# kchmck/p25rx

Measured on NVIDIA B200. Metric: Msamples/s IQ demod+decode (real-time P25 channels = baseband samples/s / 48000), higher is better.
Workload: dtype f32

## Files before the change

### p25rx_b200/csrc/ddc_fm.cu

```cuda
#include <stdlib.h>

#include "p25cu_internal.cuh"
#include "p25_imma_tables.h"

__constant__ float c_taps_front[P25_TAPS_FRONT];
__constant__ float c_taps_decim[P25_TAPS_DECIM];
__constant__ float c_taps_chan[P25_TAPS_CHAN];
__constant__ float c_iq_lut[256];

static_assert(P25_TAPS_FRONT == 5 * P25_DECIM_FRONT, "front stage is a 10-phase x 5-tap polyphase matrix");
static_assert(P25_TAPS_DECIM == 5 * P25_DECIM_NATIVE, "decimator is a 5-phase x 5-tap polyphase matrix");

template <bool FRONT>
struct Cfg {
    static constexpr int MB = FRONT ? 64 : 256;
    static constexpr int NT = FRONT ? 320 : 256;
    static constexpr int DIN = FRONT ? 50 : 5;
    static constexpr int XN = MB * DIN;
    static constexpr int ACOLS = FRONT ? 5 * MB : 0;
    static constexpr int RING = FRONT ? 128 : 512;
    static constexpr int HT = FRONT ? 3264 : 1312;
};

template <bool FRONT>
// ... 1462 lines not shown
      }
      if (it_first + n_st == ips) {
          const uint4* src = reinterpret_cast<const uint4*>(chunk + ((size_t)p.n - p.ht) * ES);
          uint4* dst = reinterpret_cast<uint4*>((unsigned char*)p.tail_out + s * tail_bytes);
          for (int i = lane; i < (int)(tail_bytes / 16); i += 32) dst[i] = src[i];
      }
      s++;
      it_first = 0;
      chunk += row_bytes;
      tail += tail_bytes;
    }
}

using Tables = p25imma::Tables5;
static_assert(NB == p25imma::NB5 && SCALE_LOG2 == p25imma::SCALE5 && sizeof(g_btab) == sizeof(Tables::b), "table geometry");
static const Tables& tables() {
    static const Tables t(P25_TAPS_DECIM_H);
    return t;
}

}


namespace w50i {

using fast::mbar_init;
using fast::mbar_expect_tx;
using fast::mbar_wait;
using fast::tma_load_1d;
using fast::cfma;
using fast5::add2;
using fast5::disc_atan2_pair;
using w5i::imma;
using w5i::imma0;
using w5i::lds32;

constexpr int D = 50;
constexpr int G = P25_TAPS_FRONT + P25_DECIM_FRONT * (P25_TAPS_DECIM - 1);
constexpr int R = 4;
constexpr int NOUT = 32 * R;
constexpr int XNEW = D * NOUT;
constexpr int XREAD = D * (NOUT - 1) + G;
constexpr int WARPS = 12;
constexpr int AL = 8, ES = 2;
constexpr int XLEN = (XREAD + 2 * AL - 2) / AL * AL;
constexpr int KS = 28;
// ... 233 lines not shown

unsigned p25cu_ddc_tail_len(int decimation) { return decimation == 50 ? Cfg<true>::HT : Cfg<false>::HT; }

cudaError_t p25cu_ddc_upload_taps() {
    cudaError_t e;
    if ((e = cudaMemcpyToSymbol(c_taps_front, P25_TAPS_FRONT_H, sizeof(c_taps_front))) != cudaSuccess) return e;
    if ((e = cudaMemcpyToSymbol(c_taps_decim, P25_TAPS_DECIM_H, sizeof(c_taps_decim))) != cudaSuccess) return e;
    if ((e = cudaMemcpyToSymbol(c_taps_chan, P25_TAPS_CHAN_H, sizeof(c_taps_chan))) != cudaSuccess) return e;
    {
        const w5i::Tables& t = w5i::tables();
        if (!t.ok) return cudaErrorInvalidValue;
        if ((e = cudaMemcpyToSymbol(w5i::g_btab, t.b, sizeof(w5i::g_btab))) != cudaSuccess) return e;
        const int4 q[3] = {make_int4(t.init[0], t.init[0], t.init[0], t.init[0]), make_int4(t.init[1], t.init[1], t.init[1], t.init[1]),
                           make_int4(t.init[2], t.init[2], t.init[2], t.init[2])};
        if ((e = cudaMemcpyToSymbol(w5i::g_init, q, sizeof(q))) != cudaSuccess) return e;
    }
    {
        const w50i::Tables& t = w50i::tables();
        if (!t.ok) return cudaErrorInvalidValue;
        if ((e = cudaMemcpyToSymbol(w50i::g_btab, t.b, sizeof(w50i::g_btab))) != cudaSuccess) return e;
        const int4 q[3] = {make_int4(t.init[0], t.init[0], t.init[0], t.init[0]), make_int4(t.init[1], t.init[1], t.init[1], t.init[1]),
                           make_int4(t.init[2], t.init[2], t.init[2], t.init[2])};
        if ((e = cudaMemcpyToSymbol(w50i::g_init, q, sizeof(q))) != cudaSuccess) return e;
    }
    return cudaMemcpyToSymbol(c_iq_lut, P25_IQ_LUT, sizeof(c_iq_lut));
}

template <bool FRONT, int FMT>
static cudaError_t launch(const DdcParams& p, cudaStream_t st) {
    using C = Cfg<FRONT>;
    auto kern = p25_ddc_fm_kernel<FRONT, FMT>;
    const size_t smem = sizeof(Smem<FRONT>);
    kern<<<p.n_streams * p.n_seg, C::NT, smem, st>>>(p);
    return cudaGetLastError();
}

unsigned p25cu_ddc_block_out(int decimation) { return decimation == 50 ? Cfg<true>::MB : Cfg<false>::MB; }

static double tap_gain(const float* h, int n) {
    double g = 0.0;
    for (int k = 0; k < n; k++) g += (double)h[k];
    return g;
}

template <int FMT>
static cudaError_t launch_fast(const DdcParams& p, cudaStream_t st) {
// ... 42 lines not shown
    const unsigned grid = want < (unsigned long long)grid_max ? (unsigned)(want ? want : 1) : (unsigned)grid_max;
    const bool u8 = FMT == P25CU_FMT_U8_IQ;
    const float dc = u8 ? (float)(0.5 * tap_gain(P25_TAPS_DECIM_H, P25_TAPS_DECIM) * tap_gain(P25_TAPS_CHAN_H, P25_TAPS_CHAN)) : 0.f;
    kern<<<grid, 32 * w5::WARPS, smem, st>>>(p, ips, dc, u8 ? (float)(1.0 / (127.5 * 127.5)) : 1.f);
    return cudaGetLastError();
}

static cudaError_t launch_w5i(const DdcParams& p, cudaStream_t st) {
    const size_t smem = sizeof(w5i::WarpSm) * w5i::WARPS + sizeof(uint2) * w5i::NB * 32;
    const unsigned ips = (p.n_out + w5i::NOUT - 1) / w5i::NOUT;
    const unsigned long long total = (unsigned long long)p.n_streams * ips;
    unsigned long long want = (total + 3) / 4;
    want = (want + w5i::WARPS - 1) / w5i::WARPS;
    const unsigned grid = want < (unsigned long long)p.plan->grid_w5i ? (unsigned)(want ? want : 1) : (unsigned)p.plan->grid_w5i;
    const w5i::Tables& t = w5i::tables();
    const double sc = (double)(1 << w5i::SCALE_LOG2);
    const float dc = (float)(0.5 * t.gain * tap_gain(P25_TAPS_CHAN_H, P25_TAPS_CHAN) * sc);
    const float pw_scale = (float)(1.0 / (127.5 * 127.5) / (sc * sc));
    if (p.power_sum) w5i::p25_ddc5_imma_kernel<true><<<grid, 32 * w5i::WARPS, smem, st>>>(p, ips, dc, pw_scale);
    else w5i::p25_ddc5_imma_kernel<false><<<grid, 32 * w5i::WARPS, smem, st>>>(p, ips, dc, pw_scale);
    return cudaGetLastError();
}

static cudaError_t launch_w50i(const DdcParams& p, cudaStream_t st) {
    const size_t smem = sizeof(w50i::WarpSm) * w50i::WARPS + sizeof(uint2) * w50i::NB * 32;
    const unsigned ips = (p.n_out + w50i::NOUT - 1) / w50i::NOUT;
    const unsigned long long total = (unsigned long long)p.n_streams * ips;
    unsigned long long want = (total + 3) / 4;
    want = (want + w50i::WARPS - 1) / w50i::WARPS;
    const unsigned grid = want < (unsigned long long)p.plan->grid_w50i ? (unsigned)(want ? want : 1) : (unsigned)p.plan->grid_w50i;
    const w50i::Tables& t = w50i::tables();
    const double sc = (double)(1 << w50i::SCALE_LOG2);
    const float dc = (float)(0.5 * t.gain * tap_gain(P25_TAPS_CHAN_H, P25_TAPS_CHAN) * sc);
    const float pw_scale = (float)(1.0 / (127.5 * 127.5) / (sc * sc));
    if (p.power_sum) w50i::p25_ddc50_imma_kernel<true><<<grid, 32 * w50i::WARPS, smem, st>>>(p, ips, dc, pw_scale);
    else w50i::p25_ddc50_imma_kernel<false><<<grid, 32 * w50i::WARPS, smem, st>>>(p, ips, dc, pw_scale);
    return cudaGetLastError();
}

template <typename K>
static cudaError_t plan_one(K kern, int threads, size_t smem, int n_sm, int* grid) {
    cudaError_t e = cudaFuncSetAttribute(kern, cudaFuncAttributeMaxDynamicSharedMemorySize, (int)smem);
    if (e != cudaSuccess) return e;
    int per_sm = 0;
    e = cudaOccupancyMaxActiveBlocksPerMultiprocessor(&per_sm, kern, threads, smem);
    if (e != cudaSuccess) return e;
// ... 6 lines not shown
    const int n_sm = plan->n_sm;
    constexpr int U8 = P25CU_FMT_U8_IQ, CF = P25CU_FMT_CF32_IQ;
    if ((e = plan_one(fast::p25_ddc_fm_stream_kernel<CF>, fast::NT, sizeof(fast::Smem<CF>), n_sm, &plan->grid_ddc50)) != cudaSuccess) return e;
    if ((e = plan_one(fast::p25_ddc_fm_stream_kernel<U8>, fast::NT, sizeof(fast::Smem<U8>), n_sm, &plan->grid_ddc50_u8)) != cudaSuccess) return e;
    if (const char* ev = getenv("P25CU_DDC_CTAS")) {
        const int per_sm = atoi(ev);
        if (per_sm > 0) plan->grid_ddc50 = plan->grid_ddc50_u8 = n_sm * per_sm;
    }
    if ((e = plan_one(fast5::p25_ddc5_fm_kernel<U8>, fast5::K<U8>::NT, sizeof(fast5::Smem<U8>), n_sm, &plan->grid_fast5[U8])) != cudaSuccess) return e;
    if ((e = plan_one(fast5::p25_ddc5_fm_kernel<CF>, fast5::K<CF>::NT, sizeof(fast5::Smem<CF>), n_sm, &plan->grid_fast5[CF])) != cudaSuccess) return e;
    if ((e = plan_one(w5::p25_ddc5_warp_kernel<U8, false>, 32 * w5::WARPS, sizeof(w5::WarpSm<U8>) * w5::WARPS, n_sm, &plan->grid_w5[U8])) != cudaSuccess) return e;
    if ((e = plan_one(w5::p25_ddc5_warp_kernel<CF, false>, 32 * w5::WARPS, sizeof(w5::WarpSm<CF>) * w5::WARPS, n_sm, &plan->grid_w5[CF])) != cudaSuccess) return e;
    if (const char* ev = getenv("P25CU_W5_CTAS")) {
        const int per_sm = atoi(ev);
        if (per_sm > 0) plan->grid_w5[U8] = plan->grid_w5[CF] = n_sm * per_sm;
    }
    const size_t smem_w5i = sizeof(w5i::WarpSm) * w5i::WARPS + sizeof(uint2) * w5i::NB * 32;
    if ((e = plan_one(w5i::p25_ddc5_imma_kernel<true>, 32 * w5i::WARPS, smem_w5i, n_sm, &plan->grid_w5i)) != cudaSuccess) return e;
    if ((e = plan_one(w5i::p25_ddc5_imma_kernel<false>, 32 * w5i::WARPS, smem_w5i, n_sm, &plan->grid_w5i)) != cudaSuccess) return e;
    if (const char* ev = getenv("P25CU_W5_CTAS")) {
        const int per_sm = atoi(ev);
        if (per_sm > 0) plan->grid_w5i = n_sm * per_sm;
    }
    const size_t smem_w50i = sizeof(w50i::WarpSm) * w50i::WARPS + sizeof(uint2) * w50i::NB * 32;
    if ((e = plan_one(w50i::p25_ddc50_imma_kernel<true>, 32 * w50i::WARPS, smem_w50i, n_sm, &plan->grid_w50i)) != cudaSuccess) return e;
    if ((e = plan_one(w50i::p25_ddc50_imma_kernel<false>, 32 * w50i::WARPS, smem_w50i, n_sm, &plan->grid_w50i)) != cudaSuccess) return e;
    const size_t atab = w5::ATAB_FLOATS * sizeof(float);
    if ((e = plan_one(w5::p25_ddc5_warp_kernel<U8, true>, 32 * w5::WARPS, sizeof(w5::WarpSm<U8, true>) * w5::WARPS + atab, n_sm, &plan->grid_w5m[U8])) != cudaSuccess) return e;
    if ((e = plan_one(w5::p25_ddc5_warp_kernel<CF, true>, 32 * w5::WARPS, sizeof(w5::WarpSm<CF, true>) * w5::WARPS + atab, n_sm, &plan->grid_w5m[CF])) != cudaSuccess) return e;
    if ((e = cudaFuncSetAttribute(p25_ddc_fm_kernel<true, U8>, cudaFuncAttributeMaxDynamicSharedMemorySize, (int)sizeof(Smem<true>))) != cudaSuccess) return e;
    if ((e = cudaFuncSetAttribute(p25_ddc_fm_kernel<true, CF>, cudaFuncAttributeMaxDynamicSharedMemorySize, (int)sizeof(Smem<true>))) != cudaSuccess) return e;
    if ((e = cudaFuncSetAttribute(p25_ddc_fm_kernel<false, U8>, cudaFuncAttributeMaxDynamicSharedMemorySize, (int)sizeof(Smem<false>))) != cudaSuccess) return e;
    return cudaFuncSetAttribute(p25_ddc_fm_kernel<false, CF>, cudaFuncAttributeMaxDynamicSharedMemorySize, (int)sizeof(Smem<false>));
}

static int ddc5_variant() {
    static const int v = getenv("P25CU_DDC5") ? atoi(getenv("P25CU_DDC5")) : 11;
    return v;
}

cudaError_t p25cu_launch_ddc(const DdcParams& p, int format, int decimation, cudaStream_t st) {
    if (p.n_out == 0 && p.n == 0) return cudaSuccess;
    if (decimation == 5 && p.aligned16 && p.n_out > 0 && p.a0 >= p.ht && p.n >= p.ht && p.ht == (unsigned)Cfg<false>::HT) {
        const bool mma = (ddc5_variant() & 4) != 0;
        if (format == P25CU_FMT_U8_IQ && (ddc5_variant() & 8)) return launch_w5i(p, st);
        if (format == P25CU_FMT_U8_IQ && (ddc5_variant() & 1))
            return mma ? launch_w5<P25CU_FMT_U8_IQ, true>(p, st) : launch_w5<P25CU_FMT_U8_IQ, false>(p, st);
        if (format == P25CU_FMT_CF32_IQ && (ddc5_variant() & 2))
            return mma ? launch_w5<P25CU_FMT_CF32_IQ, true>(p, st) : launch_w5<P25CU_FMT_CF32_IQ, false>(p, st);
    }
    if (decimation == 5 && p.aligned16 && p.n_out > 0 && p.a0 >= p.ht && p.n >= p.ht && p.ht == (unsigned)Cfg<false>::HT)
        return format == P25CU_FMT_CF32_IQ ? launch_fast5<P25CU_FMT_CF32_IQ>(p, st) : launch_fast5<P25CU_FMT_U8_IQ>(p, st);
    if (decimation == 50 && format == P25CU_FMT_CF32_IQ && p.aligned16 && (p.a0 & 1ull) == 0 && p.n_out > 0 &&
        p.ht == (unsigned)Cfg<true>::HT)
        return launch_fast<P25CU_FMT_CF32_IQ>(p, st);
    if (decimation == 50 && format == P25CU_FMT_U8_IQ && p.aligned16 && p.n_out > 0 && p.a0 >= p.ht && p.ht == (unsigned)Cfg<true>::HT) {
        static const int v50 = getenv("P25CU_DDC50") ? atoi(getenv("P25CU_DDC50")) : 1;
        if ((v50 & 1) && p.n >= p.ht) return launch_w50i(p, st);
        return launch_fast<P25CU_FMT_U8_IQ>(p, st);
    }
    if (decimation == 50)
        return format == P25CU_FMT_CF32_IQ ? launch<true, P25CU_FMT_CF32_IQ>(p, st) : launch<true, P25CU_FMT_U8_IQ>(p, st);
    return format == P25CU_FMT_CF32_IQ ? launch<false, P25CU_FMT_CF32_IQ>(p, st) : launch<false, P25CU_FMT_U8_IQ>(p, st);
}
```

### p25rx_b200/csrc/p25_imma_tables.h

```cpp
#pragma once
#include <math.h>

#include "p25_tables.h"

namespace p25imma {

struct Frag {
    unsigned x, y;
};

constexpr int MAGIC = 0x4B400000;

inline bool split_limbs(long long t, int (&d)[3]) {
    long long v = t;
    for (int l = 0; l < 3; l++) {
        const long long q = ((v + 128) & 255) - 128;
        d[l] = (int)q;
        v = (v - q) / 256;
    }
    return v == 0;
}

constexpr int NB5 = 18, SCALE5 = 25;
struct Tables5 {
// ... 68 lines not shown
            if (128 * asum[l] >= (1 << 22)) ok = false;
        gain = (double)tsum / (double)(1 << SCALE50);
        for (int l = 0; l < 3; l++) init[l] = MAGIC - 128 * (int)sum[l];
        for (int sk = 0; sk < 2; sk++)
            for (int ks = 0; ks < KS50; ks++)
                for (int l = 0; l < 3; l++)
                    for (int ln = 0; ln < 32; ln++) {
                        const int n = ln >> 2, tig = ln & 3;
                        unsigned w[2] = {0u, 0u};
                        for (int h = 0; h < 2; h++)
                            for (int bb = 0; bb < 4; bb++) {
                                const int phi = 32 * ks + 16 * h + 4 * tig + bb;
                                const int smp = phi >> 1, comp = phi & 1;
                                const int d = smp - sk - 50 * (n >> 1);
                                int v = 0;
                                if (comp == (n & 1) && d >= 0 && d < G50) v = limb[G50 - 1 - d][l];
                                w[h] |= (unsigned)(v & 255) << (8 * bb);
                            }
                        b[sk][ks * 3 + l][ln] = Frag{w[0], w[1]};
                    }
    }
};

}
```

### p25rx_b200/csrc/p25cu_api.cu

```cuda
#include <math.h>
#include <stdio.h>
#include <stdlib.h>
#include <string.h>

#include <mutex>
#include <new>

#include "p25cu_internal.cuh"

unsigned p25cu_ddc_block_out(int decimation);
cudaError_t p25cu_walk_upload_consts();
unsigned p25cu_pfb_tail_len();
unsigned p25cu_pfb_channels();
unsigned p25cu_pfb_decimation();
cudaError_t p25cu_pfb_upload(float** d_taps, float2** d_twiddle);
cudaError_t p25cu_launch_pfb(const void* iq, const void* tail_in, void* tail_out, const float* taps, const float2* twiddle,
                             float2* y, unsigned y_rows, float* bb, size_t row_stride, float* power_sum,
                             unsigned long long a0, unsigned long long m0, unsigned n, unsigned n_out, unsigned n_captures,
                             cudaStream_t st, unsigned* launches, const P25DevPlan* plan);

static std::mutex g_plan_mu;
static P25DevPlan g_plans[P25CU_MAX_DEVICES];
static bool g_plan_ok[P25CU_MAX_DEVICES];

struct p25cu_ctx {
    p25cu_config cfg;
    const P25DevPlan* plan;
    cudaStream_t stream;
    cudaStream_t stream2;
    cudaStream_t stream_copy;
    cudaEvent_t ev_bb_ready[2], ev_bb_free[2];
    cudaEvent_t ev_iq_ready[2], ev_iq_free[2];
    int overlap;
    int walk_prefilter;
    char err[512];
    unsigned ht;
    size_t max_out;
    size_t row_stride;
    unsigned ev_cap;
    void* d_iq[2];
    size_t d_iq_bytes[2];
    int iq_slot;
    float2* d_tail[2];
    int tail_cur;
    float* d_bb[2];
    int bb_cur;
    int bb_last;
    float* d_power;
    unsigned* d_work;
    int timing;
    unsigned n_timed;
    cudaEvent_t tev[2 * 128];
    unsigned ticket_base;
    WalkStateHbm* d_states;
    unsigned* d_slots;
    p25cu_event* d_dense;
    unsigned* d_offsets;
// ... 109 lines not shown
            CK(p25cu_pfb_plan_device(&pl));
            g_plan_ok[cfg.device] = true;
        }
        ctx->plan = &g_plans[cfg.device];
    }
    {
        int lo = 0, hi = 0;
        CK(cudaDeviceGetStreamPriorityRange(&lo, &hi));
        const char* e = getenv("P25CU_WALK_PRIO");
        const int mode = e ? atoi(e) : 0;
        CK(cudaStreamCreateWithPriority(&ctx->stream, cudaStreamNonBlocking, mode == 1 ? lo : hi));
        CK(cudaStreamCreateWithPriority(&ctx->stream2, cudaStreamNonBlocking, mode == 0 ? lo : hi));
        CK(cudaStreamCreateWithFlags(&ctx->stream_copy, cudaStreamNonBlocking));
    }
    for (int i = 0; i < 2; i++) {
        CK(cudaEventCreateWithFlags(&ctx->ev_bb_ready[i], cudaEventDisableTiming));
        CK(cudaEventCreateWithFlags(&ctx->ev_bb_free[i], cudaEventDisableTiming));
        CK(cudaEventCreateWithFlags(&ctx->ev_iq_ready[i], cudaEventDisableTiming));
        CK(cudaEventCreateWithFlags(&ctx->ev_iq_free[i], cudaEventDisableTiming));
        CK(cudaEventCreateWithFlags(&ctx->ev_poll[i], cudaEventDisableTiming));
    }
    ctx->overlap = (cfg.decimation == 50 && cfg.format == P25CU_FMT_CF32_IQ) ? 1 : 0;
    if (const char* e = getenv("P25CU_OVERLAP")) ctx->overlap = atoi(e) ? 1 : 0;
    ctx->walk_prefilter = cfg.decimation == (int)p25cu_pfb_decimation() ? 1 : 0;
    if (const char* e = getenv("P25CU_WALK_PREFILTER")) ctx->walk_prefilter = atoi(e) ? 1 : 0;
    const size_t S = cfg.n_streams;
    const bool wide = cfg.decimation == (int)p25cu_pfb_decimation();
    ctx->n_captures = wide ? cfg.n_streams / p25cu_pfb_channels() : 0;
    ctx->ht = wide ? p25cu_pfb_tail_len() : p25cu_ddc_tail_len(cfg.decimation);
    ctx->max_out = cfg.max_chunk_samples / cfg.decimation + 1;
    if (cfg.max_baseband > ctx->max_out) ctx->max_out = cfg.max_baseband;
    ctx->row_stride = (P25CU_BB_HIST + ctx->max_out + 3) & ~(size_t)3;
    ctx->ev_cap = cfg.event_slots ? cfg.event_slots : (unsigned)(ctx->max_out / 200 + 16);

    const size_t tail_rows = wide ? ctx->n_captures : S;
    CK(cudaMalloc(&ctx->d_tail[0], tail_rows * ctx->ht * sizeof(float2)));
    CK(cudaMalloc(&ctx->d_tail[1], tail_rows * ctx->ht * sizeof(float2)));
    CK(cudaMemsetAsync(ctx->d_tail[0], 0, tail_rows * ctx->ht * sizeof(float2), ctx->stream));
    CK(cudaMemsetAsync(ctx->d_tail[1], 0, tail_rows * ctx->ht * sizeof(float2), ctx->stream));
    if (wide) {
        ctx->y_rows = (unsigned)ctx->max_out;
        CK(p25cu_pfb_upload(&ctx->d_pfb_taps, &ctx->d_twiddle));
    }
    for (int i = 0; i < 2; i++) {
        CK(cudaMalloc(&ctx->d_bb[i], S * ctx->row_stride * sizeof(float)));
        CK(cudaMemsetAsync(ctx->d_bb[i], 0, S * ctx->row_stride * sizeof(float), ctx->stream));
    }
    CK(cudaMalloc(&ctx->d_power, S * sizeof(float)));
    CK(cudaMalloc(&ctx->d_work, 64));
    CK(cudaMemsetAsync(ctx->d_work, 0, 64, ctx->stream));
    if ((unsigned long long)S * ctx->ev_cap * P25CU_SLOT_WORDS >= (1ull << 32))
        return fail_arg(ctx, "n_streams x event_slots too large (event word offsets are 32-bit): poll more often with fewer slots");
    CK(cudaMalloc(&ctx->d_states, S * sizeof(WalkStateHbm)));
    CK(cudaMemsetAsync(ctx->d_states, 0, S * sizeof(WalkStateHbm), ctx->stream));
    CK(cudaMalloc(&ctx->d_slots, S * ctx->ev_cap * P25CU_SLOT_WORDS * sizeof(unsigned)));
// ... 80 lines not shown
        CK(cudaStreamWaitEvent(ctx->stream, ctx->ev_iq_ready[slot], 0));
        d_in = ctx->d_iq[slot];
    }
    const unsigned D = (unsigned)ctx->cfg.decimation;
    DdcParams p;
    memset(&p, 0, sizeof p);
    p.plan = ctx->plan;
    p.iq = d_in;
    p.tail_in = ctx->d_tail[ctx->tail_cur];
    p.tail_out = ctx->d_tail[ctx->tail_cur ^ 1];
    const int buf = ctx->bb_cur;
    CK(cudaStreamWaitEvent(ctx->stream, ctx->ev_bb_free[buf], 0));
    p.bb = ctx->d_bb[buf];
    p.row_stride = ctx->row_stride;
    p.power_sum = power_dbm ? ctx->d_power : nullptr;
    p.a0 = ctx->a_abs;
    p.m0 = ctx->a_abs / D;
    p.n = (unsigned)n;
    p.n_out = (unsigned)((ctx->a_abs + n) / D - p.m0);
    p.n_streams = (unsigned)S;
    p.ht = ctx->ht;
    p.work_counter = ctx->d_work;
    p.ticket_base = &ctx->ticket_base;
    p.aligned16 = ((n % (ctx->cfg.format == P25CU_FMT_U8_IQ ? 8 : 2)) == 0) && (((uintptr_t)d_in & 15) == 0);
    {
        const unsigned mb = p25cu_ddc_block_out(D);
        const unsigned iters = (p.n_out + mb - 1) / mb;
        unsigned want = (unsigned)((size_t)ctx->n_sm * 16 / S);
        unsigned cap = iters / 8;
        if (want > cap) want = cap;
        if (want < 1) want = 1;
        const unsigned per = (iters + want - 1) / want;
        p.seg_out = (per ? per : 1) * mb;
        p.n_seg = p.n_out ? (p.n_out + p.seg_out - 1) / p.seg_out : 1;
    }
    if (power_dbm) CK(cudaMemsetAsync(ctx->d_power, 0, S * sizeof(float), ctx->stream));
    const bool timed = ctx->timing && n && ctx->n_timed < 128;
    if (timed) CK(cudaEventRecord(ctx->tev[2 * ctx->n_timed], ctx->stream));
    if (n && ctx->n_captures) {
        const size_t ch = p25cu_pfb_channels();
        unsigned nl = 0;
        if (ctx->keep_spectra && !ctx->d_y) CK(cudaMalloc(&ctx->d_y, (size_t)ctx->n_captures * ctx->y_rows * ch * sizeof(float2)));
        CK(p25cu_launch_pfb(d_in, p.tail_in, p.tail_out, ctx->d_pfb_taps, ctx->d_twiddle, ctx->keep_spectra ? ctx->d_y : nullptr,
                            ctx->y_rows, p.bb, p.row_stride, p.power_sum, p.a0, p.m0, p.n, p.n_out, ctx->n_captures, ctx->stream, &nl,
                            ctx->plan));
        ctx->launches += nl;
// ... 438 lines not shown
```

### p25rx_b200/csrc/p25cu_internal.cuh

```cuda
#pragma once
#include <cuda_runtime.h>
#include <stdint.h>

#include "../../include/p25cu.h"
#include "p25_fec.cuh"

#define P25CU_BB_HIST 256
#define P25CU_MAX_DEVICES 64
#define P25CU_WALK_WARPS 2
#define P25CU_SLOT_WORDS 20
#define P25CU_BUF_DIBITS 848

enum { WS_SYNC = 0, WS_NID = 1, WS_PAYLOAD = 2, WS_FLUSH = 3 };

struct __align__(16) WalkHeader {
    unsigned long long next_sym;
    unsigned long long pos;
    int state, duid, cnt, blocks, part, chunks;
    int have_prev, prev_above;
    float prev_corr, pth, mid, nth;
    unsigned frame_pos;
    unsigned n_events;
    unsigned n_words;
    unsigned overflow;
// ... 20 lines not shown
    unsigned long long p0;
    unsigned n;
    unsigned n_streams;
    WalkStateHbm* states;
    unsigned* slots;
    unsigned ev_cap;
    unsigned long long* stats;
    const P25DevTables* tables;
    float* bb_next;
};

__host__ __device__ inline unsigned p25cu_packed_words(unsigned len) { return 3u + ((len + 3u) >> 2); }

struct P25DevPlan {
    int device;
    int n_sm;
    int grid_ddc50;
    int grid_ddc50_u8;
    int grid_fast5[2];
    int grid_w5[2];
    int grid_w5m[2];
    int grid_w50i;
    int grid_w5i;
    int pfb_slots;
};

struct DdcParams {
    const P25DevPlan* plan;
    const void* iq;
    const void* tail_in;
    void* tail_out;
    float* bb;
    size_t row_stride;
    float* power_sum;
    unsigned long long a0;
    unsigned long long m0;
    unsigned n;
    unsigned n_out;
    unsigned n_streams;
    unsigned seg_out;
    unsigned n_seg;
    unsigned ht;
    int aligned16;
    unsigned* work_counter;
    unsigned* ticket_base;
};

cudaError_t p25cu_launch_ddc(const DdcParams& p, int format, int decimation, cudaStream_t st);
cudaError_t p25cu_ddc_upload_taps();
unsigned p25cu_ddc_tail_len(int decimation);
cudaError_t p25cu_ddc_plan_device(P25DevPlan* plan);
cudaError_t p25cu_pfb_plan_device(P25DevPlan* plan);
cudaError_t p25cu_launch_walk(const WalkParams& p, cudaStream_t st, unsigned max_blocks, int device, bool prefilter);
cudaError_t p25cu_launch_compact(WalkStateHbm* states, const unsigned* slots, unsigned ev_cap, unsigned n_streams,
                                 unsigned* offsets, int mode, p25cu_event* dense80, unsigned* packed, unsigned long long cap_words,
                                 unsigned* totals_out, cudaStream_t st);
cudaError_t p25cu_launch_fec_selftest(const P25DevTables* tables, int kind, void* words, size_t count, int n, int k,
                                      void* out_data, int32_t* out_nerr, cudaStream_t st);
```

Measured before the change: 760,600.

## Add tcgen05 UMMA decimate-by-5 DDC kernel with TMA ring and TMEM accumulators

Adds a Blackwell tcgen05-based int8 UMMA kernel for the decimate-by-5 path. It folds the decimator and channel filter into one combined tap set split into three int8 limbs, streams swizzled IQ atoms through a 9-deep TMA ring, and double-buffers accumulators in tensor memory. Dedicated producer, MMA and epilogue warps handle the FM discriminator and boxcar. It becomes the default variant via P25CU_DDC5_DEFAULT, and row stride is padded to 8 floats for 32-byte vector stores. The gain is meant to come from moving the FIR dot products off per-warp IMMA onto the larger tcgen05 MMA with an async pipeline, at the cost of complexity and a timeout/abort path.

```diff
diff --git a/p25rx_b200/csrc/ddc_fm.cu b/p25rx_b200/csrc/ddc_fm.cu
--- a/p25rx_b200/csrc/ddc_fm.cu
+++ b/p25rx_b200/csrc/ddc_fm.cu
@@ -1,4 +1,8 @@
+#include <stdio.h>
 #include <stdlib.h>
+
+#include <cuda.h>
+#include <cudaTypedefs.h>
 
 #include "p25cu_internal.cuh"
 #include "p25_imma_tables.h"
@@ -1508,6 +1512,338 @@
 }
 
 
+namespace w5t {
+
+using fast::smem_u32;
+using fast::mbar_init;
+using fast::mbar_expect_tx;
+using fast::cfma;
+using fast5::add2;
+using fast5::disc_atan2_pair;
+
+constexpr int M = 128;
+constexpr int NOUT = p25imma::NOUTT;
+constexpr int N = p25imma::NT_COLS;
+constexpr int KB = p25imma::KBT;
+constexpr int KSTEPS = KB / 32;
+constexpr int ADV = 2 * 5 * NOUT;
+constexpr int ATOM = 128 * M;
+constexpr int BSLICE = 128 * N;
+constexpr int BBYTES = p25imma::BT_BYTES;
+constexpr int NA = 9;
+constexpr int EPI = 8, NT = 32 * (EPI + 2);
+constexpr int HALF = NOUT / 2;
+constexpr int NACC = 2;
+constexpr int TMEM_COLS = NACC * N <= 256 ? 256 : 512;
+constexpr int SCALE_LOG2 = p25imma::SCALET;
+constexpr int XD_BYTES = 2 * 2 * HALF * M * 4;
+constexpr size_t SMEM = 1024 + (size_t)NA * ATOM + BBYTES + XD_BYTES + 256;
+static_assert(KSTEPS * 32 == KB && BBYTES == (KB + 127) / 128 * BSLICE, "window");
+static_assert(ADV % 32 == 0 && (KB + 96 + 127) / 128 <= NA - 3, "K steps stay in their atom; ring depth");
+static_assert(NACC * N <= TMEM_COLS && N % 16 == 0 && N == 3 * 32, "accumulators");
+
+__device__ unsigned char g_btab[p25imma::PHASES_T][BBYTES];
+__device__ int g_init[3];
+
+__device__ __forceinline__ void wait(unsigned long long* bar, unsigned parity, volatile int* abort_flag) {
+    unsigned ok;
+    unsigned long long t0 = 0;
+    for (int spin = 0;; spin++) {
+        asm volatile(
+            "{\n\t.reg .pred p;\n\tmbarrier.try_wait.parity.shared::cta.b64 p, [%1], %2;\n\tselp.u32 %0, 1, 0, p;\n\t}"
+            : "=r"(ok)
+            : "r"(smem_u32(bar)), "r"(parity)
+            : "memory");
+        if (ok) return;
+        if ((spin & 1023) == 1023) {
+            unsigned long long t;
+            asm volatile("mov.u64 %0, %%globaltimer;" : "=l"(t));
+            if (!t0) t0 = t;
+            if (*abort_flag) return;
+            if (t - t0 > 4000000000ull) {
+                printf("w5t: mbarrier timeout, block %d thread %d barrier smem+%u parity %u\n", blockIdx.x, threadIdx.x,
+                       smem_u32(bar), parity);
+                *abort_flag = 1;
+                return;
+            }
+        }
+    }
+}
+
+__device__ __forceinline__ void mbar_arrive(unsigned long long* bar) {
+    asm volatile("mbarrier.arrive.shared::cta.b64 _, [%0];" ::"r"(smem_u32(bar)) : "memory");
+}
+
+__device__ __forceinline__ void tma_2d(unsigned dst, const CUtensorMap* map, int x, int y, unsigned long long* bar) {
+    asm volatile("cp.async.bulk.tensor.2d.shared::cluster.global.mbarrier::complete_tx::bytes [%0], [%1, {%2, %3}], [%4];" ::"r"(dst),
+                 "l"(reinterpret_cast<unsigned long long>(map)), "r"(x), "r"(y), "r"(smem_u32(bar))
+                 : "memory");
+}
+
+__device__ __forceinline__ unsigned long long sdesc(unsigned addr) {
+    return (unsigned long long)((addr & 0x3FFFFu) >> 4) | ((unsigned long long)(1024 >> 4) << 32) | (1ull << 46) | (2ull << 61);
+}
+constexpr unsigned IDESC = (2u << 4) | (0u << 7) | (1u << 10) | ((unsigned)(N >> 3) << 17) | ((unsigned)(M >> 4) << 24);
+
+__device__ __forceinline__ void umma(unsigned tmem, unsigned long long a, unsigned long long b, unsigned acc) {
+    asm volatile("{\n\t.reg .pred p;\n\tsetp.ne.b32 p, %4, 0;\n\t"
+                 "tcgen05.mma.cta_group::1.kind::i8 [%0], %1, %2, %3, p;\n\t}" ::"r"(tmem), "l"(a), "l"(b), "r"(IDESC), "r"(acc));
+}
+__device__ __forceinline__ bool elect_one() {
+    unsigned r;
+    asm volatile("{\n\t.reg .pred p;\n\telect.sync _|p, 0xffffffff;\n\tselp.u32 %0, 1, 0, p;\n\t}" : "=r"(r));
+    return r != 0;
+}
+__device__ __forceinline__ void umma_commit(unsigned long long* bar) {
+    asm volatile("tcgen05.commit.cta_group::1.mbarrier::arrive::one.shared::cluster.b64 [%0];" ::"r"(smem_u32(bar)) : "memory");
+}
+__device__ __forceinline__ void tmem_ld16(unsigned taddr, unsigned (&r)[16]) {
+    asm volatile("tcgen05.ld.sync.aligned.32x32b.x16.b32 {%0,%1,%2,%3,%4,%5,%6,%7,%8,%9,%10,%11,%12,%13,%14,%15}, [%16];"
+                 : "=r"(r[0]), "=r"(r[1]), "=r"(r[2]), "=r"(r[3]), "=r"(r[4]), "=r"(r[5]), "=r"(r[6]), "=r"(r[7]), "=r"(r[8]),
+                   "=r"(r[9]), "=r"(r[10]), "=r"(r[11]), "=r"(r[12]), "=r"(r[13]), "=r"(r[14]), "=r"(r[15])
+                 : "r"(taddr));
+}
+__device__ __forceinline__ void tmem_ld2(unsigned taddr, unsigned (&r)[2]) {
+    asm volatile("tcgen05.ld.sync.aligned.32x32b.x2.b32 {%0,%1}, [%2];" : "=r"(r[0]), "=r"(r[1]) : "r"(taddr));
+}
+
+__device__ __forceinline__ int win_start(int p_bytes, int it) { return (p_bytes + ADV * it) & ~31; }
+
+template <bool PW>
+__global__ void __launch_bounds__(NT, 1) p25_ddc5_umma_kernel(const __grid_constant__ CUtensorMap tm_chunk,
+                                                            const __grid_constant__ CUtensorMap tm_tail, const DdcParams p,
+                                                            const unsigned its_per_tile, const float dc, const float pw_scale) {
+    extern __shared__ unsigned char smem_raw[];
+    const unsigned sbase = (smem_u32(smem_raw) + 1023u) & ~1023u;
+    unsigned char* const gbase = smem_raw + (sbase - smem_u32(smem_raw));
+    const unsigned sa = sbase, sb = sbase + NA * ATOM;
+    unsigned long long* const full = reinterpret_cast<unsigned long long*>(gbase + NA * ATOM + BBYTES + XD_BYTES);
+    unsigned long long* const empty = full + NA;
+    unsigned long long* const tfull = empty + NA;
+    unsigned long long* const tempty = tfull + NACC;
+    unsigned* const tslot = reinterpret_cast<unsigned*>(tempty + NACC);
+    volatile int* const abort_flag = reinterpret_cast<volatile int*>(tslot + 1);
+    const int warp = threadIdx.x >> 5, lane = threadIdx.x & 31;
+
+    const int ips = (int)its_per_tile, n_out = (int)p.n_out, S = (int)p.n_streams;
+    const int p_bytes = 2 * ((int)(5 * (long long)p.m0 - (long long)p.a0) - (p25imma::GT - 5));
+    const int phase = ((p_bytes & 31) >> 1);
+    {
+        const uint4* src = reinterpret_cast<const uint4*>(g_btab[phase]);
+        uint4* dst = reinterpret_cast<uint4*>(gbase + NA * ATOM);
+        for (int i = threadIdx.x; i < BBYTES / 16; i += NT) dst[i] = src[i];
+    }
+    if (threadIdx.x == 0) {
+        for (int i = 0; i < NA; i++) {
+            mbar_init(&full[i], 1);
+            mbar_init(&empty[i], 1);
+        }
+        for (int i = 0; i < NACC; i++) {
+            mbar_init(&tfull[i], 1);
+            mbar_init(&tempty[i], 32 * EPI);
+        }
+        *abort_flag = 0;
+        asm volatile("fence.mbarrier_init.release.cluster;" ::: "memory");
+    }
+    if (warp == 0) {
+        asm volatile("tcgen05.alloc.cta_group::1.sync.aligned.shared::cta.b32 [%0], %1;" ::"r"(smem_u32(tslot)), "r"(TMEM_COLS));
+        asm volatile("tcgen05.relinquish_alloc_permit.cta_group::1.sync.aligned;");
+    }
+    asm volatile("fence.proxy.async.shared::cta;" ::: "memory");
+    asm volatile("tcgen05.fence::before_thread_sync;" ::: "memory");
+    __syncthreads();
+    asm volatile("tcgen05.fence::after_thread_sync;" ::: "memory");
+    const unsigned tmem = *tslot;
+
+    const unsigned long long total = (unsigned long long)((S + M - 1) / M) * (unsigned)ips;
+    const unsigned long long w0 = total * blockIdx.x / gridDim.x, w1 = total * (blockIdx.x + 1ull) / gridDim.x;
+
+    if (warp == EPI && lane == 0) {
+        unsigned q = 0;
+        for (unsigned long long w = w0; w < w1;) {
+            const int tile = (int)(w / ips), itf = (int)(w % ips);
+            const int n_st = (int)min((unsigned long long)(ips - itf), w1 - w);
+            w += n_st;
+            const int a_first = win_start(p_bytes, itf - 1) >> 7, a_last = (win_start(p_bytes, itf + n_st - 1) + KB - 1) >> 7;
+            for (int a = a_first; a <= a_last; a++, q++) {
+                const unsigned slot = q % NA;
+                if (q >= NA) wait(&empty[slot], (q / NA - 1) & 1, abort_flag);
+                mbar_expect_tx(&full[slot], ATOM);
+                if (a >= 0) tma_2d(sa + slot * ATOM, &tm_chunk, 128 * a, M * tile, &full[slot]);
+                else tma_2d(sa + slot * ATOM, &tm_tail, 2 * (int)p.ht + 128 * a, M * tile, &full[slot]);
+            }
+        }
+    } else if (warp == EPI + 1) {
+        const bool leader = elect_one();
+        const unsigned long long a_desc = sdesc(sa), b_desc = sdesc(sb);
+        unsigned q_base = 0, q_ready = 0, q_rel = 0, u = 0;
+        for (unsigned long long w = w0; w < w1;) {
+            const int itf = (int)(w % ips);
+            const int n_st = (int)min((unsigned long long)(ips - itf), w1 - w);
+            w += n_st;
+            const int a_first = win_start(p_bytes, itf - 1) >> 7, a_last = (win_start(p_bytes, itf + n_st - 1) + KB - 1) >> 7;
+            for (int j = 0; j <= n_st; j++, u++) {
+                const int it = itf - 1 + j;
+                const int g0 = win_start(p_bytes, it);
+                const unsigned need = q_base + (unsigned)(((g0 + KB - 1) >> 7) - a_first);
+                for (; q_ready <= need; q_ready++) wait(&full[q_ready % NA], (q_ready / NA) & 1, abort_flag);
+                const unsigned buf = u % NACC;
+                if (u >= NACC) wait(&tempty[buf], (u / NACC - 1) & 1, abort_flag);
+                __syncwarp();
+                asm volatile("tcgen05.fence::after_thread_sync;" ::: "memory");
+                const unsigned q0 = q_base + (unsigned)((g0 >> 7) - a_first), off0 = (unsigned)g0 & 127u;
+                const int keep = j < n_st ? (win_start(p_bytes, it + 1) >> 7) : a_last + 1;
+                const unsigned rel_end = q_base + (unsigned)(keep - a_first);
+                if (leader) {
+#pragma unroll
+                    for (int k = 0; k < KSTEPS; k++) {
+                        const unsigned off = off0 + 32u * k, slot = (q0 + (off >> 7)) % NA;
+                        umma(tmem + buf * N, a_desc + ((slot * ATOM + (off & 127u)) >> 4), b_desc + (((k >> 2) * BSLICE + (k & 3) * 32) >> 4), k);
+                    }
+                    umma_commit(&tfull[buf]);
+                    for (unsigned q = q_rel; q < rel_end; q++) umma_commit(&empty[q % NA]);
+                }
+                q_rel = rel_end;
+                __syncwarp();
+            }
+            q_base += (unsigned)(a_last - a_first + 1);
+        }
+    } else if (warp < EPI) {
+        const int h = warp >> 2, row = 32 * (warp & 3) + lane;
+        const unsigned taddr0 = tmem + ((unsigned)(32 * (warp & 3)) << 16);
+        const unsigned col_own = 16u * h, col_extra = h ? 14u : 30u;
+        const int init0 = g_init[0], init1 = g_init[1], init2 = g_init[2];
+        const size_t row_bytes = (size_t)p.n * 2, tail_bytes = (size_t)p.ht * 2;
+        float* const xd = reinterpret_cast<float*>(gbase + NA * ATOM + BBYTES);
+        unsigned u = 0;
+        float2 c_carry = make_float2(0.f, 0.f);
+        float d_carry = 0.f;
+        for (unsigned long long w = w0; w < w1;) {
+            const int tile = (int)(w / ips), itf = (int)(w % ips);
+            const int n_st = (int)min((unsigned long long)(ips - itf), w1 - w);
+            w += n_st;
+            const int s = M * tile + row;
+            const bool live = s < S;
+            float* const out_row = p.bb + (size_t)(live ? s : 0) * p.row_stride + P25CU_BB_HIST + HALF * h;
+            float pw = 0.f;
+            for (int j = 0; j <= n_st; j++, u++) {
+                const int it = itf - 1 + j;
+                const unsigned buf = u % NACC;
+                float hist[HALF];
+                if (h == 0) {
+#pragma unroll
+                    for (int k = 0; k < HALF; k++) hist[k] = xd[((((u + 1) & 1) * 2 + 1) * HALF + k) * M + row];
+                }
+                wait(&tfull[buf], (u / NACC) & 1, abort_flag);
+                __syncwarp();
+                asm volatile("tcgen05.fence::after_thread_sync;" ::: "memory");
+                float2 c[HALF], cx;
+                {
+                    const int init[3] = {init0, init1, init2};
+                    unsigned r[3][2 * HALF], rx[3][2];
+#pragma unroll
+                    for (int l = 0; l < 3; l++) {
+                        tmem_ld16(taddr0 + buf * N + 32 * l + col_own, r[l]);
+                        tmem_ld2(taddr0 + buf * N + 32 * l + col_extra, rx[l]);
+                    }
+                    asm volatile("tcgen05.wait::ld.sync.aligned;" ::: "memory");
+                    asm volatile("tcgen05.fence::before_thread_sync;" ::: "memory");
+                    mbar_arrive(&tempty[buf]);
+                    const float2 unmagic = make_float2(-12582912.f, -12582912.f);
+                    auto limb = [&](unsigned a, unsigned b, int l) {
+                        return add2(make_float2(__int_as_float((int)a + init[l]), __int_as_float((int)b + init[l])), unmagic);
+                    };
+#pragma unroll
+                    for (int o = 0; o < HALF; o++) {
+                        const float2 f0 = limb(r[0][2 * o], r[0][2 * o + 1], 0), f1 = limb(r[1][2 * o], r[1][2 * o + 1], 1),
+                                     f2 = limb(r[2][2 * o], r[2][2 * o + 1], 2);
+                        c[o] = add2(cfma(65536.f, f2, cfma(256.f, f1, f0)), make_float2(dc, dc));
+                    }
+                    const float2 f0 = limb(rx[0][0], rx[0][1], 0), f1 = limb(rx[1][0], rx[1][1], 1), f2 = limb(rx[2][0], rx[2][1], 2);
+                    cx = add2(cfma(65536.f, f2, cfma(256.f, f1, f0)), make_float2(dc, dc));
+                }
+                const int nv = j ? min(n_out - NOUT * it, NOUT) - HALF * h : 0;
+                float dd[HALF];
+                float2 prev = h ? cx : c_carry;
+#pragma unroll
+                for (int o = 0; o < HALF; o += 2) {
+                    const float2 c0 = c[o], c1 = c[o + 1];
+                    const float2 re = make_float2(c0.x * prev.x + c0.y * prev.y, c1.x * c0.x + c1.y * c0.y);
+                    const float2 im = make_float2(c0.y * prev.x - c0.x * prev.y, c1.y * c0.x - c1.x * c0.y);
+                    const float2 th = disc_atan2_pair(im, re);
+                    dd[o] = th.x * P25_FM_GAIN;
+                    dd[o + 1] = th.y * P25_FM_GAIN;
+                    if (PW && o < nv) pw += c0.x * c0.x + c0.y * c0.y;
+                    if (PW && o + 1 < nv) pw += c1.x * c1.x + c1.y * c1.y;
+                    prev = c1;
+                }
+                if (h == 0) c_carry = cx;
+#pragma unroll
+                for (int k = 0; k < HALF; k++) xd[(((u & 1) * 2 + h) * HALF + k) * M + row] = dd[k];
+                asm volatile("bar.sync 1, %0;" ::"r"(32 * EPI) : "memory");
+                if (h == 1) {
+#pragma unroll
+                    for (int k = 0; k < HALF; k++) hist[k] = xd[(((u & 1) * 2) * HALF + k) * M + row];
+                }
+                float sum[HALF];
+                {
+                    float s0 = d_carry + hist[0];
+#pragma unroll
+                    for (int k = 1; k < HALF; k++) s0 += hist[k];
+                    sum[0] = s0 + dd[0];
+                    sum[1] = (sum[0] - d_carry) + dd[1];
+#pragma unroll
+                    for (int o = 2; o < HALF; o++) sum[o] = (sum[o - 1] - hist[o - 2]) + dd[o];
+                }
+                d_carry = dd[HALF - 1];
+                if (live && nv > 0) {
+                    const float kk = 1.0f / P25_BOXCAR;
+                    float* const out = out_row + NOUT * it;
+                    if (nv >= HALF && !((uintptr_t)out & 31)) {
+                        asm volatile("st.global.v8.f32 [%0], {%1,%2,%3,%4,%5,%6,%7,%8};" ::"l"(out), "f"(sum[0] * kk), "f"(sum[1] * kk),
+                                     "f"(sum[2] * kk), "f"(sum[3] * kk), "f"(sum[4] * kk), "f"(sum[5] * kk), "f"(sum[6] * kk),
+                                     "f"(sum[7] * kk)
+                                     : "memory");
+                    } else if (nv >= HALF) {
+                        reinterpret_cast<float4*>(out)[0] = make_float4(sum[0] * kk, sum[1] * kk, sum[2] * kk, sum[3] * kk);
+                        reinterpret_cast<float4*>(out)[1] = make_float4(sum[4] * kk, sum[5] * kk, sum[6] * kk, sum[7] * kk);
+                    } else {
+#pragma unroll
+                        for (int o = 0; o < HALF; o++)
+                            if (o < nv) out[o] = sum[o] * kk;
+                    }
+                }
+            }
+            if (PW && live) atomicAdd(p.power_sum + s, pw * pw_scale);
+            if (itf + n_st == ips) {
+                const int rows = min(M, S - M * tile), per_row = (int)(tail_bytes / 16);
+                const unsigned char* src = (const unsigned char*)p.iq + (size_t)M * tile * row_bytes + (row_bytes - tail_bytes);
+                unsigned char* dst = (unsigned char*)p.tail_out + (size_t)M * tile * tail_bytes;
+                for (int i = threadIdx.x; i < rows * per_row; i += 32 * EPI) {
+                    const int r = i / per_row, k = i - r * per_row;
+                    reinterpret_cast<uint4*>(dst + r * tail_bytes)[k] = reinterpret_cast<const uint4*>(src + r * row_bytes)[k];
+                }
+            }
+        }
+    }
+    asm volatile("tcgen05.fence::before_thread_sync;" ::: "memory");
+    __syncthreads();
+    if (warp == 0) {
+        asm volatile("tcgen05.fence::after_thread_sync;" ::: "memory");
+        asm volatile("tcgen05.dealloc.cta_group::1.sync.aligned.b32 %0, %1;" ::"r"(tmem), "r"(TMEM_COLS));
+    }
+}
+
+using Tables = p25imma::TablesT;
+static_assert(sizeof(g_btab) == sizeof(Tables::b), "table geometry");
+static const Tables& tables() {
+    static const Tables t(P25_TAPS_DECIM_H, P25_TAPS_CHAN_H);
+    return t;
+}
+
+}
+
+
 namespace w50i {
 
 using fast::mbar_init;
@@ -1787,6 +2123,12 @@
         const int4 q[3] = {make_int4(t.init[0], t.init[0], t.init[0], t.init[0]), make_int4(t.init[1], t.init[1], t.init[1], t.init[1]),
                            make_int4(t.init[2], t.init[2], t.init[2], t.init[2])};
         if ((e = cudaMemcpyToSymbol(w50i::g_init, q, sizeof(q))) != cudaSuccess) return e;
+    }
+    {
+        const w5t::Tables& t = w5t::tables();
+        if (!t.ok) return cudaErrorInvalidValue;
+        if ((e = cudaMemcpyToSymbol(w5t::g_btab, t.b, sizeof(w5t::g_btab))) != cudaSuccess) return e;
+        if ((e = cudaMemcpyToSymbol(w5t::g_init, t.init, sizeof(w5t::g_init))) != cudaSuccess) return e;
     }
     return cudaMemcpyToSymbol(c_iq_lut, P25_IQ_LUT, sizeof(c_iq_lut));
 }
@@ -1875,6 +2217,48 @@
     return cudaGetLastError();
 }
 
+static PFN_cuTensorMapEncodeTiled_v12000 tensor_map_encoder() {
+    static const PFN_cuTensorMapEncodeTiled_v12000 fn = [] {
+        void* f = nullptr;
+        cudaDriverEntryPointQueryResult q;
+        if (cudaGetDriverEntryPointByVersion("cuTensorMapEncodeTiled", &f, 12000, cudaEnableDefault, &q) != cudaSuccess ||
+            q != cudaDriverEntryPointSuccess)
+            f = nullptr;
+        return reinterpret_cast<PFN_cuTensorMapEncodeTiled_v12000>(f);
+    }();
+    return fn;
+}
+
+static cudaError_t u8_atom_map(CUtensorMap* m, const void* base, unsigned long long width, unsigned rows) {
+    const PFN_cuTensorMapEncodeTiled_v12000 enc = tensor_map_encoder();
+    if (!enc) return cudaErrorNotSupported;
+    const cuuint64_t dims[2] = {width, rows};
+    const cuuint64_t strides[1] = {width};
+    const cuuint32_t box[2] = {128, (cuuint32_t)w5t::M};
+    const cuuint32_t estr[2] = {1, 1};
+    const CUresult r = enc(m, CU_TENSOR_MAP_DATA_TYPE_UINT8, 2, const_cast<void*>(base), dims, strides, box, estr,
+                           CU_TENSOR_MAP_INTERLEAVE_NONE, CU_TENSOR_MAP_SWIZZLE_128B, CU_TENSOR_MAP_L2_PROMOTION_L2_256B,
+                           CU_TENSOR_MAP_FLOAT_OOB_FILL_NONE);
+    return r == CUDA_SUCCESS ? cudaSuccess : cudaErrorInvalidValue;
+}
+
+static cudaError_t launch_w5t(const DdcParams& p, cudaStream_t st) {
+    const unsigned ipt = (p.n_out + w5t::NOUT - 1) / w5t::NOUT;
+    const unsigned long long total = (unsigned long long)((p.n_streams + w5t::M - 1) / w5t::M) * ipt;
+    const unsigned grid = total < (unsigned long long)p.plan->grid_w5t ? (unsigned)total : (unsigned)p.plan->grid_w5t;
+    CUtensorMap tm_chunk, tm_tail;
+    cudaError_t e;
+    if ((e = u8_atom_map(&tm_chunk, p.iq, 2ull * p.n, p.n_streams)) != cudaSuccess) return e;
+    if ((e = u8_atom_map(&tm_tail, p.tail_in, 2ull * p.ht, p.n_streams)) != cudaSuccess) return e;
+    const w5t::Tables& t = w5t::tables();
+    const double sc = (double)(1 << w5t::SCALE_LOG2);
+    const float dc = (float)(0.5 * t.gain * sc);
+    const float pw_scale = (float)(1.0 / (127.5 * 127.5) / (sc * sc));
+    if (p.power_sum) w5t::p25_ddc5_umma_kernel<true><<<grid, w5t::NT, w5t::SMEM, st>>>(tm_chunk, tm_tail, p, ipt, dc, pw_scale);
+    else w5t::p25_ddc5_umma_kernel<false><<<grid, w5t::NT, w5t::SMEM, st>>>(tm_chunk, tm_tail, p, ipt, dc, pw_scale);
+    return cudaGetLastError();
+}
+
 static cudaError_t launch_w50i(const DdcParams& p, cudaStream_t st) {
     const size_t smem = sizeof(w50i::WarpSm) * w50i::WARPS + sizeof(uint2) * w50i::NB * 32;
     const unsigned ips = (p.n_out + w50i::NOUT - 1) / w50i::NOUT;
@@ -1927,6 +2311,8 @@
         const int per_sm = atoi(ev);
         if (per_sm > 0) plan->grid_w5i = n_sm * per_sm;
     }
+    if ((e = plan_one(w5t::p25_ddc5_umma_kernel<true>, w5t::NT, w5t::SMEM, n_sm, &plan->grid_w5t)) != cudaSuccess) return e;
+    if ((e = plan_one(w5t::p25_ddc5_umma_kernel<false>, w5t::NT, w5t::SMEM, n_sm, &plan->grid_w5t)) != cudaSuccess) return e;
     const size_t smem_w50i = sizeof(w50i::WarpSm) * w50i::WARPS + sizeof(uint2) * w50i::NB * 32;
     if ((e = plan_one(w50i::p25_ddc50_imma_kernel<true>, 32 * w50i::WARPS, smem_w50i, n_sm, &plan->grid_w50i)) != cudaSuccess) return e;
     if ((e = plan_one(w50i::p25_ddc50_imma_kernel<false>, 32 * w50i::WARPS, smem_w50i, n_sm, &plan->grid_w50i)) != cudaSuccess) return e;
@@ -1939,19 +2325,16 @@
     return cudaFuncSetAttribute(p25_ddc_fm_kernel<false, CF>, cudaFuncAttributeMaxDynamicSharedMemorySize, (int)sizeof(Smem<false>));
 }
 
-static int ddc5_variant() {
-    static const int v = getenv("P25CU_DDC5") ? atoi(getenv("P25CU_DDC5")) : 11;
-    return v;
-}
-
 cudaError_t p25cu_launch_ddc(const DdcParams& p, int format, int decimation, cudaStream_t st) {
     if (p.n_out == 0 && p.n == 0) return cudaSuccess;
     if (decimation == 5 && p.aligned16 && p.n_out > 0 && p.a0 >= p.ht && p.n >= p.ht && p.ht == (unsigned)Cfg<false>::HT) {
-        const bool mma = (ddc5_variant() & 4) != 0;
-        if (format == P25CU_FMT_U8_IQ && (ddc5_variant() & 8)) return launch_w5i(p, st);
-        if (format == P25CU_FMT_U8_IQ && (ddc5_variant() & 1))
+        const int v = p.ddc5_variant;
+        const bool mma = (v & 4) != 0;
+        if (format == P25CU_FMT_U8_IQ && (v & 16)) return launch_w5t(p, st);
+        if (format == P25CU_FMT_U8_IQ && (v & 8)) return launch_w5i(p, st);
+        if (format == P25CU_FMT_U8_IQ && (v & 1))
             return mma ? launch_w5<P25CU_FMT_U8_IQ, true>(p, st) : launch_w5<P25CU_FMT_U8_IQ, false>(p, st);
-        if (format == P25CU_FMT_CF32_IQ && (ddc5_variant() & 2))
+        if (format == P25CU_FMT_CF32_IQ && (v & 2))
             return mma ? launch_w5<P25CU_FMT_CF32_IQ, true>(p, st) : launch_w5<P25CU_FMT_CF32_IQ, false>(p, st);
     }
     if (decimation == 5 && p.aligned16 && p.n_out > 0 && p.a0 >= p.ht && p.n >= p.ht && p.ht == (unsigned)Cfg<false>::HT)
diff --git a/p25rx_b200/csrc/p25_imma_tables.h b/p25rx_b200/csrc/p25_imma_tables.h
--- a/p25rx_b200/csrc/p25_imma_tables.h
+++ b/p25rx_b200/csrc/p25_imma_tables.h
@@ -114,4 +114,53 @@
     }
 };
 
+constexpr int GT = P25_TAPS_DECIM + P25_DECIM_NATIVE * (P25_TAPS_CHAN - 1);
+constexpr int NOUTT = 16, NT_COLS = NOUTT * 2 * 3, KBT = 608, PHASES_T = P25_DECIM_NATIVE, SCALET = 27;
+constexpr int BT_BYTES = (KBT + 127) / 128 * 128 * NT_COLS;
+static_assert(2 * (PHASES_T - 1 + P25_DECIM_NATIVE * (NOUTT - 1) + GT) <= KBT, "every phase's window inside K");
+
+inline int sw128_offset(int rows, int row, int kbyte) {
+    const int slice = kbyte >> 7, chunk = (kbyte >> 4) & 7;
+    return slice * rows * 128 + (row >> 3) * 1024 + (row & 7) * 128 + ((chunk ^ (row & 7)) << 4) + (kbyte & 15);
 }
+
+struct TablesT {
+    unsigned char b[PHASES_T][BT_BYTES];
+    int init[3];
+    double gain;
+    bool ok;
+    TablesT(const float* hd, const float* hc) {
+        static_assert(P25_TAPS_DECIM == 25 && P25_DECIM_NATIVE == 5, "geometry");
+        double g[GT];
+        for (int j = 0; j < GT; j++) g[j] = 0.0;
+        for (int k = 0; k < P25_TAPS_CHAN; k++)
+            for (int e = 0; e < P25_TAPS_DECIM; e++) g[P25_DECIM_NATIVE * k + e] += (double)hc[k] * (double)hd[e];
+        static int limb[GT][3];
+        long long sum[3] = {0, 0, 0}, asum[3] = {0, 0, 0}, tsum = 0;
+        ok = true;
+        for (int j = 0; j < GT; j++) {
+            const long long t = llround(g[j] * (double)(1 << SCALET));
+            if (!split_limbs(t, limb[j])) ok = false;
+            for (int l = 0; l < 3; l++) {
+                sum[l] += limb[j][l];
+                asum[l] += limb[j][l] < 0 ? -limb[j][l] : limb[j][l];
+            }
+            tsum += t;
+        }
+        for (int l = 0; l < 3; l++)
+            if (128 * asum[l] >= (1 << 22)) ok = false;
+        gain = (double)tsum / (double)(1 << SCALET);
+        for (int l = 0; l < 3; l++) init[l] = MAGIC - 128 * (int)sum[l];
+        for (int ph = 0; ph < PHASES_T; ph++)
+            for (int n = 0; n < NT_COLS; n++)
+                for (int kb = 0; kb < BT_BYTES / NT_COLS; kb++) {
+                    const int l = n >> 5, jo = (n & 31) >> 1, c = n & 1;
+                    const int d = (kb >> 1) - ph - P25_DECIM_NATIVE * jo;
+                    int v = 0;
+                    if ((kb & 1) == c && d >= 0 && d < GT) v = limb[GT - 1 - d][l];
+                    b[ph][sw128_offset(NT_COLS, n, kb)] = (unsigned char)(v & 255);
+                }
+    }
+};
+
+}
diff --git a/p25rx_b200/csrc/p25cu_api.cu b/p25rx_b200/csrc/p25cu_api.cu
--- a/p25rx_b200/csrc/p25cu_api.cu
+++ b/p25rx_b200/csrc/p25cu_api.cu
@@ -33,6 +33,7 @@
     cudaEvent_t ev_iq_ready[2], ev_iq_free[2];
     int overlap;
     int walk_prefilter;
+    int ddc5_variant;
     char err[512];
     unsigned ht;
     size_t max_out;
@@ -188,6 +189,8 @@
     }
     ctx->overlap = (cfg.decimation == 50 && cfg.format == P25CU_FMT_CF32_IQ) ? 1 : 0;
     if (const char* e = getenv("P25CU_OVERLAP")) ctx->overlap = atoi(e) ? 1 : 0;
+    ctx->ddc5_variant = P25CU_DDC5_DEFAULT;
+    if (const char* e = getenv("P25CU_DDC5")) ctx->ddc5_variant = atoi(e);
     ctx->walk_prefilter = cfg.decimation == (int)p25cu_pfb_decimation() ? 1 : 0;
     if (const char* e = getenv("P25CU_WALK_PREFILTER")) ctx->walk_prefilter = atoi(e) ? 1 : 0;
     const size_t S = cfg.n_streams;
@@ -196,7 +199,7 @@
     ctx->ht = wide ? p25cu_pfb_tail_len() : p25cu_ddc_tail_len(cfg.decimation);
     ctx->max_out = cfg.max_chunk_samples / cfg.decimation + 1;
     if (cfg.max_baseband > ctx->max_out) ctx->max_out = cfg.max_baseband;
-    ctx->row_stride = (P25CU_BB_HIST + ctx->max_out + 3) & ~(size_t)3;
+    ctx->row_stride = (P25CU_BB_HIST + ctx->max_out + 7) & ~(size_t)7;
     ctx->ev_cap = cfg.event_slots ? cfg.event_slots : (unsigned)(ctx->max_out / 200 + 16);
 
     const size_t tail_rows = wide ? ctx->n_captures : S;
@@ -323,6 +326,7 @@
     p.ht = ctx->ht;
     p.work_counter = ctx->d_work;
     p.ticket_base = &ctx->ticket_base;
+    p.ddc5_variant = ctx->ddc5_variant;
     p.aligned16 = ((n % (ctx->cfg.format == P25CU_FMT_U8_IQ ? 8 : 2)) == 0) && (((uintptr_t)d_in & 15) == 0);
     {
         const unsigned mb = p25cu_ddc_block_out(D);
diff --git a/p25rx_b200/csrc/p25cu_internal.cuh b/p25rx_b200/csrc/p25cu_internal.cuh
--- a/p25rx_b200/csrc/p25cu_internal.cuh
+++ b/p25rx_b200/csrc/p25cu_internal.cuh
@@ -66,6 +66,7 @@
     int grid_w5m[2];
     int grid_w50i;
     int grid_w5i;
+    int grid_w5t;
     int pfb_slots;
 };
 
@@ -88,7 +89,10 @@
     int aligned16;
     unsigned* work_counter;
     unsigned* ticket_base;
+    int ddc5_variant;
 };
+
+#define P25CU_DDC5_DEFAULT 27
 
 cudaError_t p25cu_launch_ddc(const DdcParams& p, int format, int decimation, cudaStream_t st);
 cudaError_t p25cu_ddc_upload_taps();
diff --git a/spec/w5t_dataflow.py b/spec/w5t_dataflow.py
--- /dev/null
+++ b/spec/w5t_dataflow.py
@@ -0,0 +1,127 @@
+from __future__ import annotations
+
+import numpy as np
+
+M, NOUT, N, KB, PHASES, SCALE = 128, 16, 96, 608, 5, 27
+KSTEPS = KB // 32
+GT = 225
+ADV = 160
+NA_RING = 9
+ATOM = 128 * M
+BSLICE = 128 * N
+BT_BYTES = (KB + 127) // 128 * BSLICE
+MAGIC = 0x4B400000
+
+
+def combined_taps(hd: np.ndarray, hc: np.ndarray) -> np.ndarray:
+    g = np.zeros(len(hd) + 5 * (len(hc) - 1))
+    for k, h in enumerate(hc.astype(np.float64)):
+        g[5 * k: 5 * k + len(hd)] += h * hd.astype(np.float64)
+    return g
+
+
+def limbs(g: np.ndarray):
+    out = np.zeros((len(g), 3), dtype=np.int64)
+    t = np.zeros(len(g), dtype=np.int64)
+    for j, h in enumerate(g):
+        v = t[j] = int(np.round(float(h) * (1 << SCALE)))
+        for l in range(3):
+            d = ((v + 128) & 255) - 128
+            out[j, l] = d
+            v = (v - d) // 256
+        assert v == 0, "tap does not fit 24 bits"
+    return out, t
+
+
+def sw128(rows: int, row: int, kbyte: int) -> int:
+    return (kbyte >> 7) * rows * 128 + (row >> 3) * 1024 + (row & 7) * 128 + ((((kbyte >> 4) & 7) ^ (row & 7)) << 4) + (kbyte & 15)
+
+
+def column(l: int, j: int, c: int) -> int:
+    return 32 * l + 2 * j + c
+
+
+def b_operand(lb: np.ndarray, phase: int) -> np.ndarray:
+    out = np.zeros(BT_BYTES, dtype=np.int64)
+    for l in range(3):
+        for j in range(NOUT):
+            for c in range(2):
+                n = column(l, j, c)
+                for d in range(GT):
+                    kb = 2 * (phase + 5 * j + d) + c
+                    assert kb < KB
+                    out[sw128(N, n, kb)] = lb[GT - 1 - d, l]
+    return out
+
+
+def tma_atom(x: np.ndarray, col: int) -> np.ndarray:
+    out = np.zeros(ATOM, dtype=np.int64)
+    rows, width = x.shape
+    for r in range(M):
+        for i in range(128):
+            if r < rows and 0 <= col + i < width:
+                out[sw128(M, r, i)] = x[r, col + i]
+    return out
+
+
+def umma_read(smem: np.ndarray, start: int, rows: int) -> np.ndarray:
+    r = np.arange(rows)[:, None]
+    i = np.arange(32)[None, :]
+    addr = start + (r >> 3) * 1024 + (r & 7) * 128 + i
+    return smem[addr ^ (((addr >> 7) & 7) << 4)]
+
+
+def win_start(p_bytes: int, it: int) -> int:
+    return (p_bytes + ADV * it) & ~31
+
+
+def iteration(tail: np.ndarray, chunk: np.ndarray, p_bytes: int, it: int, lb: np.ndarray, init):
+    NA = NA_RING
+    ht2 = tail.shape[1]
+    phase = (p_bytes & 31) >> 1
+    g0 = win_start(p_bytes, it)
+    a_first, a_last = g0 >> 7, (g0 + KB - 1) >> 7
+    smem = np.zeros(NA * ATOM + BT_BYTES, dtype=np.int64)
+    for q, a in enumerate(range(a_first, a_last + 1)):
+        if a >= 0:
+            img = tma_atom(chunk, 128 * a)
+        else:
+            assert ht2 + 128 * a >= 0 and ht2 + 128 * (a + 1) <= ht2, "a tail atom lies inside the tail"
+            img = tma_atom(tail, ht2 + 128 * a)
+        smem[(q % NA) * ATOM: (q % NA + 1) * ATOM] = img
+    bop = b_operand(lb, phase)
+    smem[NA * ATOM:] = bop
+    acc = np.zeros((M, N), dtype=np.int64)
+    starts = []
+    for k in range(KSTEPS):
+        byte = g0 + 32 * k
+        slot = ((byte >> 7) - a_first) % NA
+        sa = slot * ATOM + (byte & 127)
+        sb = NA * ATOM + (k >> 2) * BSLICE + (k & 3) * 32
+        assert (byte & 127) + 32 <= 128 and sa % 32 == 0
+        starts.append((sa, sb))
+        A = umma_read(smem, sa, M)
+        B = umma_read(smem, sb, N)
+        acc += A @ B.T
+    f = []
+    for l in range(3):
+        bits = (acc[:, 32 * l: 32 * l + 32] + init[l]).astype(np.int64)
+        assert np.all(np.abs(bits - MAGIC) < (1 << 22)), "sums leave the magic number's binade"
+        f.append((bits.astype(np.uint32).view(np.float32) - np.float32(12582912.0)).astype(np.float32))
+    inner = (np.float64(f[1]) * 256.0 + np.float64(f[0])).astype(np.float32)
+    y = (np.float64(f[2]) * 65536.0 + np.float64(inner)).astype(np.float32)
+    c = y[:, 0::2] + 1j * y[:, 1::2].astype(np.float64)
+    return c, starts
+
+
+def two_stage(x: np.ndarray, start: int, hd: np.ndarray, hc: np.ndarray, n_out: int) -> np.ndarray:
+    hd64, hc64 = hd.astype(np.float64), hc.astype(np.float64)
+    out = np.zeros(n_out, dtype=np.complex128)
+    for o in range(n_out):
+        acc = 0.0
+        for k in range(len(hc)):
+            q = o - k
+            base = start + 200 + 5 * q
+            acc += hc64[k] * np.dot(hd64, x[base + 24 - np.arange(len(hd))])
+        out[o] = acc
+    return out
```

Result: no change. 760,700, median of 6 (+0.0%).
